# thu-ml/zhusuan

Measured on NVIDIA H100. Metric: leapfrog-steps*chains/sec, higher is better.
Workload: dtype f32

## Files before the change

zhusuan_b200/csrc/hmc_dense_res.cu:

```cuda
#include "hmc_dense_epilogue.cuh"

namespace {

struct ResEpi {
  const __half* __restrict__ hi_cur; const __half* __restrict__ lo_cur;
  __half* __restrict__ hi_nxt; __half* __restrict__ lo_nxt;
  const __half* __restrict__ hi_cur_s; const __half* __restrict__ lo_cur_s;
  __half* __restrict__ hi_nxt_s; __half* __restrict__ lo_nxt_s;
  const float* __restrict__ p_in; float* __restrict__ p_out;
  float* __restrict__ lp_part; float* __restrict__ k_part;
  int64_t chains; int D;
  float sq, inv_sq, acc_scale;
  float rescale;
};

template <int MODE, int NEXT, int DC, bool SPARE>
__device__ __forceinline__ void epilogue_planes(const ResEpi& a, uint32_t trow, int n, bool n_ok,
                                                int64_t c0, int64_t part_row, int lane, float s2,
                                                float eps_over_m_sq, float inv_m, float b_n,
                                                float mu_n, float& qmax) {
  constexpr int NCOL = BN;
  const uint32_t D = DC ? (uint32_t)DC : (uint32_t)a.D;
  const int64_t chains = a.chains;
  const bool warp_n_ok = __all_sync(0xffffffffu, n_ok);
  const bool fast_tile = warp_n_ok && (c0 + NCOL <= chains);
  const int64_t off_t = c0 * (int64_t)D + n;
  const float* __restrict__ pin0 = a.p_in + off_t;
  float* __restrict__ po0 = a.p_out + off_t;
  const unsigned short* __restrict__ hc0 =
      reinterpret_cast<const unsigned short*>(a.hi_cur) + off_t;
  const unsigned short* __restrict__ lc0 =
      reinterpret_cast<const unsigned short*>(a.lo_cur) + off_t;
  __half* __restrict__ hn0 = NEXT ? a.hi_nxt + off_t : nullptr;
  __half* __restrict__ ln0 = NEXT ? a.lo_nxt + off_t : nullptr;
  __half* __restrict__ hs0 = SPARE ? a.hi_nxt_s + off_t : nullptr;
  __half* __restrict__ ls0 = SPARE ? a.lo_nxt_s + off_t : nullptr;

  auto element = [&](float acc, float p, uint32_t hl, float& pn, float& lpv, float& kv,
                     float& Qn) {
    const float Q = __half2float(__ushort_as_half((unsigned short)(hl & 0xFFFFu))) +
                    __half2float(__ushort_as_half((unsigned short)(hl >> 16)));
    const float g = b_n - a.acc_scale * acc;
    pn = fmaf(s2, g, p);
    if (MODE >= 1) lpv = (Q * a.inv_sq - mu_n) * g;
    if (MODE >= 2) kv = pn * pn * inv_m;
    if (NEXT) Qn = fmaf(eps_over_m_sq, pn, Q);
  };

  if (fast_tile) {
    auto load = [&](float* pe, uint32_t* he, int c) {
      const size_t cb = (size_t)c * D;
#pragma unroll
      for (int j = 0; j < 16; ++j) {
        pe[j] = __ldcg(pin0 + cb + (uint32_t)j * D);
        const uint32_t h = __ldcg(hc0 + cb + (uint32_t)j * D);
        const uint32_t l = __ldcg(lc0 + cb + (uint32_t)j * D);
        he[j] = h | (l << 16);
      }
    };
    float ss_a = 0.f, ss_b = 0.f;
    auto compute = [&](const uint32_t* v, const float* pe, const uint32_t* he, int c, float& ss) {
      const size_t cb = (size_t)c * D;
      float lpv[MODE >= 1 ? 16 : 1], kv[MODE >= 2 ? 16 : 1];
#pragma unroll
      for (int j = 0; j < 16; j += 2) {
        float pn[2], lp1[2] = {0.f, 0.f}, k1[2] = {0.f, 0.f}, Qn[2] = {0.f, 0.f};
#pragma unroll
        for (int t = 0; t < 2; ++t) {
          element(__uint_as_float(v[j + t]), pe[j + t], he[j + t], pn[t], lp1[t], k1[t], Qn[t]);
          po0[cb + (uint32_t)(j + t) * D] = pn[t];
          if (MODE >= 1) lpv[j + t] = lp1[t];
          if (MODE >= 2) kv[j + t] = k1[t];
          if (NEXT && !SPARE) ss = fmaf(Qn[t], Qn[t], ss);
          if (SPARE) qmax = fmaxf(qmax, fabsf(Qn[t]));
        }
        if (NEXT) {
          const __half2 h2 = __floats2half2_rn(Qn[0], Qn[1]);
          const float2 hf = __half22float2(h2);
          const __half2 l2 = __floats2half2_rn(Qn[0] - hf.x, Qn[1] - hf.y);
          hn0[cb + (uint32_t)j * D] = __low2half(h2);
          hn0[cb + (uint32_t)(j + 1) * D] = __high2half(h2);
          ln0[cb + (uint32_t)j * D] = __low2half(l2);
          ln0[cb + (uint32_t)(j + 1) * D] = __high2half(l2);
        }
        if (SPARE) {
          const float x0 = Qn[0] * a.rescale, x1 = Qn[1] * a.rescale;
          const __half2 h2 = __floats2half2_rn(x0, x1);
          const float2 hf = __half22float2(h2);
          const __half2 l2 = __floats2half2_rn(x0 - hf.x, x1 - hf.y);
          hs0[cb + (uint32_t)j * D] = __low2half(h2);
          hs0[cb + (uint32_t)(j + 1) * D] = __high2half(h2);
          ls0[cb + (uint32_t)j * D] = __low2half(l2);
          ls0[cb + (uint32_t)(j + 1) * D] = __high2half(l2);
        }
      }
      if (MODE >= 1) {
        const float sum = warp_transpose_sum16(lpv, lane);
        if (lane < 16) a.lp_part[part_row + c0 + c + lane] = sum;
      }
      if (MODE >= 2) {
        const float sum = warp_transpose_sum16(kv, lane);
        if (lane < 16) a.k_part[part_row + c0 + c + lane] = sum;
      }
    };
    float pa[16], pb[16];
    uint32_t ha[16], hb[16], va[16], vb[16];
    load(pa, ha, 0);
#pragma unroll 1
    for (int c = 0; c < NCOL; c += 32) {
      load(pb, hb, c + 16);
      acc_ld16(trow + 4u * (uint32_t)c, va);
      compute(va, pa, ha, c, ss_a);
      if (c + 32 < NCOL) load(pa, ha, c + 32);
      acc_ld16(trow + 4u * (uint32_t)(c + 16), vb);
      compute(vb, pb, hb, c + 16, ss_b);
    }
    if (NEXT && !SPARE) {
      const float norm = sqrtf(ss_a + ss_b) * (1.f + 0x1p-10f);
      qmax = fmaxf(qmax, norm == norm ? norm : INFINITY);
    }
  } else {
#pragma unroll 1
    for (int c = 0; c < NCOL; c += 16) {
      uint32_t v[16];
      acc_ld16(trow + 4u * (uint32_t)c, v);
      const int64_t cbase = c0 + c;
      if (cbase < chains) {
        const size_t cb = (size_t)c * D;
        float lpv[MODE >= 1 ? 16 : 1], kv[MODE >= 2 ? 16 : 1];
#pragma unroll
        for (int j = 0; j < 16; ++j) {
          const bool ok = n_ok && cbase + j < chains;
          float p = 0.f;
          uint32_t hl = 0u;
          if (ok) {
            p = __ldcg(pin0 + cb + (uint32_t)j * D);
            hl = (uint32_t)__ldcg(hc0 + cb + (uint32_t)j * D) |
                 ((uint32_t)__ldcg(lc0 + cb + (uint32_t)j * D) << 16);
          }
          float pn, lp1 = 0.f, k1 = 0.f, Qn = 0.f;
          element(__uint_as_float(v[j]), p, hl, pn, lp1, k1, Qn);
          const __half hh = __float2half_rn(Qn);
          const __half ll = __float2half_rn(Qn - __half2float(hh));
          if (NEXT && ok) qmax = fmaxf(qmax, fabsf(Qn));
          if (MODE >= 1) lpv[j] = ok ? lp1 : 0.f;
          if (MODE >= 2) kv[j] = ok ? k1 : 0.f;
          if (ok) {
            po0[cb + (uint32_t)j * D] = pn;
            if (NEXT) {
              hn0[cb + (uint32_t)j * D] = hh;
              ln0[cb + (uint32_t)j * D] = ll;
            }
            if (SPARE) {
              const float x = Qn * a.rescale;
              const __half hs = __float2half_rn(x);
              hs0[cb + (uint32_t)j * D] = hs;
              ls0[cb + (uint32_t)j * D] = __float2half_rn(x - __half2float(hs));
            }
          }
        }
        if (MODE >= 1) {
          const float sum = warp_transpose_sum16(lpv, lane);
          if (lane < 16 && cbase + lane < chains) a.lp_part[part_row + cbase + lane] = sum;
        }
        if (MODE >= 2) {
          const float sum = warp_transpose_sum16(kv, lane);
          if (lane < 16 && cbase + lane < chains) a.k_part[part_row + cbase + lane] = sum;
        }
      }
    }
  }
}


__device__ __forceinline__ int& producer_spare_in() {
  __shared__ int spare_in;
  return spare_in;
}

template <int MODE, int NEXT, int DC, int CX, int CY>
struct ResW {
  static constexpr int KIND = 1, RB = 64, MNA = 0, MNB = 0;
  static constexpr int CLUSTER = CX * CY;
  static constexpr int KE = RB / 2;
  static constexpr uint32_t TX = Cfg<RB>::STAGE;
  CUtensorMap m_phi, m_plo, m_qhi, m_qlo, m_shi, m_slo;
  ResEpi ea;
  const float* bvec; const float* mu; const float* mass; const float* state;
  float* scales;
  float p_scale;
  int n_blk, D_rt, pass;
  struct EpiState { float qmax = 0.f; };

  __device__ __forceinline__ int D() const { return DC ? DC : D_rt; }
  __host__ __device__ __forceinline__ int64_t units() const {
    return ((ea.chains + BN - 1) / BN) * (int64_t)n_blk;
  }
  __device__ __forceinline__ void tile(int64_t u, int& nb, int64_t& cb) const {
    const uint64_t cu = (uint64_t)u / CLUSTER;
    const int r = (int)((uint64_t)u % CLUSTER);
    const uint32_t nbx = (uint32_t)(n_blk / CX);
    nb = (int)(cu % nbx) * CX + r % CX;
    cb = (int64_t)(cu / nbx) * CY + r / CX;
  }
  __device__ __forceinline__ void kb_range(int64_t, int& kb0, int& kb1) const {
    kb0 = 0;
    kb1 = D() / KE;
  }
  __device__ __forceinline__ void prefetch() const {
    tma_prefetch_desc(&m_phi); tma_prefetch_desc(&m_plo);
    tma_prefetch_desc(&m_qhi); tma_prefetch_desc(&m_qlo);
    tma_prefetch_desc(&m_shi); tma_prefetch_desc(&m_slo);
    producer_spare_in() = plane_spare_in(scales, pass);
  }
  __device__ __forceinline__ void load(int64_t u, int kb, uint32_t sa, uint32_t fb) const {
    using C = Cfg<RB>;
    int nb;
    int64_t cb;
    tile(u, nb, cb);
    const int n0 = nb * BM;
    const int c0 = (int)cb * BN;
    const bool s = producer_spare_in() != 0;
    const CUtensorMap* qh = s ? &m_shi : &m_qhi;
    const CUtensorMap* ql = s ? &m_slo : &m_qlo;
    const int r = (int)(u % CLUSTER), rx = r % CX, ry = r / CX;
    if constexpr (CY == 1) {
      tma_load_2d(sa, &m_phi, fb, kb * KE, n0);
      tma_load_2d(sa + C::A_TILE, &m_plo, fb, kb * KE, n0);
    } else {
      constexpr int rows = BM / CY;
      uint16_t mask = 0;
#pragma unroll
      for (int y = 0; y < CY; ++y) mask |= (uint16_t)(1u << (y * CX + rx));
      const uint32_t o = (uint32_t)(ry * rows * RB);
      tma_load_2d_mc(sa + o, &m_phi, fb, kb * KE, n0 + ry * rows, mask);
      tma_load_2d_mc(sa + C::A_TILE + o, &m_plo, fb, kb * KE, n0 + ry * rows, mask);
    }
    if constexpr (CX == 1) {
      tma_load_2d(sa + 2 * C::A_TILE, qh, fb, kb * KE, c0);
      tma_load_2d(sa + 2 * C::A_TILE + C::B_TILE, ql, fb, kb * KE, c0);
    } else {
      constexpr int rows = BN / CX;
      const uint16_t mask = (uint16_t)(((1u << CX) - 1u) << (ry * CX));
      const uint32_t o = (uint32_t)(rx * rows * RB);
      tma_load_2d_mc(sa + 2 * C::A_TILE + o, qh, fb, kb * KE, c0 + rx * rows, mask);
      tma_load_2d_mc(sa + 2 * C::A_TILE + C::B_TILE + o, ql, fb, kb * KE, c0 + rx * rows, mask);
    }
  }
  __device__ __forceinline__ float sq_alt(float eps, float sq) const {
    return next_plane_scale(scales, pass, eps, mul(eps, p_scale), sq);
  }
  __device__ __forceinline__ void epilogue(int64_t u, uint32_t trow, int quarter, int lane,
                                           EpiState& st) const {
    int nb;
    int64_t cb;
    tile(u, nb, cb);
    const int n = nb * BM + quarter * 32 + lane;
    const int64_t c0 = cb * BN;
    const bool n_ok = n < D();
    const float eps = state[ZSB_ST_EPS_USED];
    const float s2 = mul(eps, p_scale);
    const bool spare_in = plane_spare_in(scales, pass);
    const float sq = plane_scale_in(scales, pass);
    const float m_n = n_ok ? mass[n] : 1.f;
    const float eps_over_m_sq = mul(fdiv(eps, m_n), sq);
    const float inv_m = fdiv(1.f, m_n);
    const float b_n = (n_ok && bvec) ? bvec[n] : 0.f;
    const float mu_n = (n_ok && mu) ? mu[n] : 0.f;
    const int64_t part_row = (int64_t)(nb * 4 + quarter) * ea.chains;
    ResEpi a = ea;
    if (spare_in) {
      a.hi_cur = ea.hi_cur_s;
      a.lo_cur = ea.lo_cur_s;
    }
    a.sq = sq;
    a.inv_sq = fdiv(1.f, sq);
    a.acc_scale = 1.f / (scales[3] * sq);
    a.rescale = NEXT ? sq_alt(eps, sq) * a.inv_sq : 1.f;
    if (a.rescale == 1.f)
      epilogue_planes<MODE, NEXT, DC, false>(a, trow, n, n_ok, c0, part_row, lane, s2,
                                             eps_over_m_sq, inv_m, b_n, mu_n, st.qmax);
    else
      epilogue_planes<MODE, NEXT, DC, true>(a, trow, n, n_ok, c0, part_row, lane, s2,
                                            eps_over_m_sq, inv_m, b_n, mu_n, st.qmax);
  }
  __device__ __forceinline__ void epi_finish(EpiState& st, int quarter, int lane) const {
    if (!NEXT) return;
    const float sq = plane_scale_in(scales, pass);
    const float alt = sq_alt(state[ZSB_ST_EPS_USED], sq);
    publish_plane_scale(scales, pass, sq, alt, st.qmax * (1.f / sq),
                        alt != sq && !(st.qmax < kHalfOverflow), quarter, lane);
  }
};

constexpr int RES_CX = 2, RES_CY = 2;

template <int DC, int CX, int CY>
int res_pass(const CUtensorMap& phi, const CUtensorMap& plo, const CUtensorMap& qhi,
             const CUtensorMap& qlo, const CUtensorMap& shi, const CUtensorMap& slo,
             const ResEpi& ea, const float* bvec, const float* mu, const float* mass,
             const float* state, float* scales, int pass, float p_scale, int n_blk, int D,
             int mode, cudaStream_t st) {
  if (mode == 1) {
    const ResW<1, 1, DC, CX, CY> w{phi, plo, qhi, qlo, shi, slo, ea, bvec, mu, mass, state,
                                   scales, p_scale, n_blk, D, pass};
    return tc_launch(w, st, "hmc_dense_resident");
  }
  if (mode == 0) {
    const ResW<0, 1, DC, CX, CY> w{phi, plo, qhi, qlo, shi, slo, ea, bvec, mu, mass, state,
                                   scales, p_scale, n_blk, D, pass};
    return tc_launch(w, st, "hmc_dense_resident");
  }
  const ResW<2, 0, DC, CX, CY> w{phi, plo, qhi, qlo, shi, slo, ea, bvec, mu, mass, state, scales,
                                 p_scale, n_blk, D, pass};
  return tc_launch(w, st, "hmc_dense_resident");
}

template <int DC>
int res_pass(bool cluster, const CUtensorMap& phi, const CUtensorMap& plo, const CUtensorMap& qhi,
             const CUtensorMap& qlo, const CUtensorMap& shi, const CUtensorMap& slo,
             const ResEpi& ea, const float* bvec, const float* mu, const float* mass,
             const float* state, float* scales, int pass, float p_scale, int n_blk, int D,
             int mode, cudaStream_t st) {
  return cluster ? res_pass<DC, RES_CX, RES_CY>(phi, plo, qhi, qlo, shi, slo, ea, bvec, mu, mass,
                                                state, scales, pass, p_scale, n_blk, D, mode, st)
                 : res_pass<DC, 1, 1>(phi, plo, qhi, qlo, shi, slo, ea, bvec, mu, mass, state,
                                      scales, pass, p_scale, n_blk, D, mode, st);
}

__global__ void __launch_bounds__(256) select_planes_kernel(float* __restrict__ q,
                                                            const __half* __restrict__ planes,
                                                            const __half* __restrict__ spare,
                                                            const float* __restrict__ record,
                                                            const int32_t* __restrict__ accept,
                                                            int64_t chains, int64_t D) {
  const bool use_spare = __float_as_uint(record[3]) != 0u;
  const float inv_sq = 1.f / record[use_spare ? 1 : 0];
  if (use_spare) planes = spare;
  const int lane = threadIdx.x & 31;
  const int n8 = (int)(D >> 3);
  const int64_t wstride = (int64_t)gridDim.x * 8;
  for (int64_t c = (int64_t)blockIdx.x * 8 + (threadIdx.x >> 5); c < chains; c += wstride) {
    if (!accept[c]) continue;
    const uint4* __restrict__ hi = reinterpret_cast<const uint4*>(planes + c * D);
    const uint4* __restrict__ lo = reinterpret_cast<const uint4*>(planes + (chains + c) * D);
    float4* __restrict__ qr = reinterpret_cast<float4*>(q + c * D);
    for (int i0 = lane; i0 < n8; i0 += 128) {
      uint4 h[4], l[4];
#pragma unroll
      for (int u = 0; u < 4; ++u) {
        const int i = i0 + 32 * u;
        if (i < n8) { h[u] = __ldcs(hi + i); l[u] = __ldcs(lo + i); }
      }
#pragma unroll
      for (int u = 0; u < 4; ++u) {
        const int i = i0 + 32 * u;
        if (i < n8) {
          const uint32_t hw[4] = {h[u].x, h[u].y, h[u].z, h[u].w};
          const uint32_t lw[4] = {l[u].x, l[u].y, l[u].z, l[u].w};
          float o[8];
#pragma unroll
          for (int k = 0; k < 4; ++k) {
            const float2 hf = __half22float2(*reinterpret_cast<const __half2*>(&hw[k]));
            const float2 lf = __half22float2(*reinterpret_cast<const __half2*>(&lw[k]));
            o[2 * k] = (hf.x + lf.x) * inv_sq;
            o[2 * k + 1] = (hf.y + lf.y) * inv_sq;
          }
          qr[2 * i] = make_float4(o[0], o[1], o[2], o[3]);
          qr[2 * i + 1] = make_float4(o[4], o[5], o[6], o[7]);
        }
      }
    }
  }
}

}

int zsb_dense_res_h16_launch(void* planes0, void* planes1, void* spare0, void* spare1,
                             const float* p0, float* pw,
                             const void* P_h16, const void* P_l16, float* scales,
                             const float* bvec, const float* mu, const float* mass,
                             const float* state, float* lp0_part, float* lp1_part, float* k_part,
                             int64_t chains, int D, int L, cudaStream_t st) {
  if (D % 64 != 0 || D < 64 || L < 1 || chains <= 0 || chains >= (1LL << 31)) {
    zsb_set_error("dense_res: needs D %% 64 == 0, n_leapfrogs >= 1");
    return ZSB_ERR_INVALID;
  }
  if (planes0 == planes1 || !spare0 || !spare1 || spare0 == spare1) {
    zsb_set_error("dense_res: planes1, spare0 and spare1 must be separate work buffers");
    return ZSB_ERR_INVALID;
  }
  const int n_blk = (D + BM - 1) / BM;
  const int64_t c_blk = (chains + BN - 1) / BN;
  const bool cluster = n_blk % RES_CX == 0 && c_blk % RES_CY == 0;
  const uint32_t p_box = cluster ? BM / RES_CY : BM, q_box = cluster ? BN / RES_CX : BN;
  CUtensorMap phi, plo, qhi[2], qlo[2], shi[2], slo[2];
  int rc;
  constexpr int RB = ResW<0, 1, 0, 1, 1>::RB;
  if ((rc = make_map(&phi, P_h16, (uint64_t)D, (uint64_t)D, p_box, RB, 1))) return rc;
  if ((rc = make_map(&plo, P_l16, (uint64_t)D, (uint64_t)D, p_box, RB, 1))) return rc;
  __half* pl[2] = {reinterpret_cast<__half*>(planes0), reinterpret_cast<__half*>(planes1)};
  __half* sp[2] = {reinterpret_cast<__half*>(spare0), reinterpret_cast<__half*>(spare1)};
  const int64_t plane = chains * (int64_t)D;
  for (int b = 0; b < 2; ++b) {
    if ((rc = make_map(&qhi[b], pl[b], (uint64_t)chains, (uint64_t)D, q_box, RB, 1))) return rc;
    if ((rc = make_map(&qlo[b], pl[b] + plane, (uint64_t)chains, (uint64_t)D, q_box, RB, 1)))
      return rc;
    if ((rc = make_map(&shi[b], sp[b], (uint64_t)chains, (uint64_t)D, q_box, RB, 1))) return rc;
    if ((rc = make_map(&slo[b], sp[b] + plane, (uint64_t)chains, (uint64_t)D, q_box, RB, 1)))
      return rc;
  }
  for (int i = 0; i <= L; ++i) {
    const bool last = i == L;
    const int buf = i & 1;
    const ResEpi ea{pl[buf], pl[buf] + plane, pl[buf ^ 1], pl[buf ^ 1] + plane,
                    sp[buf], sp[buf] + plane, sp[buf ^ 1], sp[buf ^ 1] + plane,
                    i == 0 ? p0 : pw, pw, i == 0 ? lp0_part : lp1_part, k_part, chains, D,
                    1.f, 1.f, 1.f, 1.f};
    const int mode = last ? 2 : (i == 0 ? 1 : 0);
    const float p_scale = (i > 0 && !last) ? 1.f : 0.5f;
    rc = (D == 1024)
             ? res_pass<1024>(cluster, phi, plo, qhi[buf], qlo[buf], shi[buf], slo[buf], ea, bvec,
                              mu, mass, state, scales, i, p_scale, n_blk, D, mode, st)
             : res_pass<0>(cluster, phi, plo, qhi[buf], qlo[buf], shi[buf], slo[buf], ea, bvec, mu,
                           mass, state, scales, i, p_scale, n_blk, D, mode, st);
    if (rc != ZSB_OK) return rc;
  }
  return ZSB_OK;
}

int zsb_dense_select_planes_launch(float* q, const void* planes, const void* spare,
                                   const float* record, const int32_t* accept, int64_t chains,
                                   int64_t D, cudaStream_t st) {
  ZSB_REQUIRE(D % 8 == 0, "zsb_dense_select_planes: D must be a multiple of 8");
  int64_t blocks = zsb_ceil_div(chains, 8);
  if (blocks > ZSB_NUM_SMS * 16) blocks = ZSB_NUM_SMS * 16;
  if (blocks < 1) blocks = 1;
  select_planes_kernel<<<(unsigned)blocks, 256, 0, st>>>(
      q, reinterpret_cast<const __half*>(planes), reinterpret_cast<const __half*>(spare), record,
      accept, chains, D);
  return zsb_check_launch("hmc_select_planes");
}
```

zhusuan_b200/csrc/tc_common.cuh:

```cuda
#pragma once
#include "common.cuh"
#include <cuda.h>
#include <cuda_fp16.h>

namespace {

constexpr int BM = 128;
constexpr int BN = 128;
constexpr int NUM_EPI_WARPS = 4;
constexpr int PRODUCER_WARP = 4;
constexpr int EPI_WARP0 = 5;
constexpr int NUM_THREADS = 32 * (EPI_WARP0 + NUM_EPI_WARPS);
constexpr int ACC_LD = BN + 4;
constexpr int ACC_BYTES = BM * ACC_LD * 4;
constexpr int STAGE_BUDGET = 128 * 1024;
constexpr long long WAIT_TIMEOUT_CYCLES = 4000000000LL;

template <int RB>
struct Cfg {
  static constexpr int A_TILE = BM * RB;
  static constexpr int B_TILE = BN * RB;
  static constexpr int STAGE = 2 * A_TILE + 2 * B_TILE;
  static constexpr int STAGES = STAGE_BUDGET / STAGE;
  static constexpr int SMEM = STAGES * STAGE + ACC_BYTES + 128 + 1024;
};

__device__ __forceinline__ uint32_t smem_u32(const void* p) {
  return (uint32_t)__cvta_generic_to_shared(p);
}
__device__ __forceinline__ void mbar_init(uint32_t bar, uint32_t count) {
  asm volatile("mbarrier.init.shared::cta.b64 [%0], %1;" ::"r"(bar), "r"(count) : "memory");
}
__device__ __forceinline__ void mbar_expect_tx(uint32_t bar, uint32_t bytes) {
  asm volatile("mbarrier.arrive.expect_tx.shared::cta.b64 _, [%0], %1;" ::"r"(bar), "r"(bytes)
               : "memory");
}
__device__ __forceinline__ void mbar_arrive(uint32_t bar) {
  asm volatile("mbarrier.arrive.shared::cta.b64 _, [%0];" ::"r"(bar) : "memory");
}
__device__ __forceinline__ bool mbar_try_wait(uint32_t bar, uint32_t parity) {
  uint32_t ok;
  asm volatile(
      "{\n\t.reg .pred P1;\n\t"
      "mbarrier.try_wait.parity.shared::cta.b64 P1, [%1], %2;\n\t"
      "selp.b32 %0, 1, 0, P1;\n\t}"
      : "=r"(ok)
      : "r"(bar), "r"(parity)
      : "memory");
  return ok != 0;
}
__device__ __forceinline__ void mbar_wait(uint32_t bar, uint32_t parity) {
  if (mbar_try_wait(bar, parity)) return;
  const long long t0 = clock64();
  while (!mbar_try_wait(bar, parity))
    if (clock64() - t0 > WAIT_TIMEOUT_CYCLES) __trap();
}
__device__ __forceinline__ void mbar_spin(uint32_t bar, uint32_t parity) {
  while (!mbar_try_wait(bar, parity)) {
  }
}
__device__ __forceinline__ void tma_load_2d(uint32_t dst, const CUtensorMap* map, uint32_t bar,
                                            int c0, int c1) {
  asm volatile(
      "cp.async.bulk.tensor.2d.shared::cluster.global.mbarrier::complete_tx::bytes"
      " [%0], [%1, {%3, %4}], [%2];"
      ::"r"(dst), "l"(map), "r"(bar), "r"(c0), "r"(c1)
      : "memory");
}
__device__ __forceinline__ void tma_load_2d_mc(uint32_t dst, const CUtensorMap* map, uint32_t bar,
                                               int c0, int c1, uint16_t mask) {
  asm volatile(
      "cp.async.bulk.tensor.2d.shared::cluster.global.mbarrier::complete_tx::bytes"
      ".multicast::cluster [%0], [%1, {%3, %4}], [%2], %5;"
      ::"r"(dst), "l"(map), "r"(bar), "r"(c0), "r"(c1), "h"(mask)
      : "memory");
}
__device__ __forceinline__ void mbar_arrive_cluster(uint32_t bar, uint32_t cta) {
  asm volatile(
      "{\n\t.reg .b32 rb;\n\t"
      "mapa.shared::cluster.u32 rb, %0, %1;\n\t"
      "mbarrier.arrive.shared::cluster.b64 _, [rb];\n\t}"
      ::"r"(bar), "r"(cta)
      : "memory");
}
__device__ __forceinline__ void cluster_sync() {
  asm volatile("barrier.cluster.arrive.release;\n\tbarrier.cluster.wait.acquire;" ::: "memory");
}
__device__ __forceinline__ void tma_prefetch_desc(const CUtensorMap* map) {
  asm volatile("prefetch.tensormap [%0];" ::"l"(map) : "memory");
}

template <int MN, int RB>
__device__ __forceinline__ uint64_t gmma_desc(uint32_t saddr) {
  uint64_t d = (uint64_t)((saddr & 0x3FFFF) >> 4);
  if (MN) {
    d |= (uint64_t)(8192 >> 4) << 16;
    d |= (uint64_t)(1024 >> 4) << 32;
    d |= (uint64_t)1 << 62;
  } else {
    d |= (uint64_t)1 << 16;
    d |= (uint64_t)((8 * RB) >> 4) << 32;
    d |= (uint64_t)(RB == 128 ? 1 : 2) << 62;
  }
  return d;
}
__device__ __forceinline__ void wgmma_fence() {
  asm volatile("wgmma.fence.sync.aligned;" ::: "memory");
}
__device__ __forceinline__ void wgmma_commit() {
  asm volatile("wgmma.commit_group.sync.aligned;" ::: "memory");
}
template <int N>
__device__ __forceinline__ void wgmma_wait() {
  asm volatile("wgmma.wait_group.sync.aligned %0;" ::"n"(N) : "memory");
}
__device__ __forceinline__ void wgmma_tf32(float (&d)[64], uint64_t da, uint64_t db) {
  asm volatile(
      "{\n\t.reg .pred p;\n\tsetp.ne.b32 p, 1, 0;\n\t"
      "wgmma.mma_async.sync.aligned.m64n128k8.f32.tf32.tf32 {%0, %1, %2, %3, %4, %5, %6, %7, %8, %9, %10, %11, %12, %13, %14, %15, %16, %17, %18, %19, %20, %21, %22, %23, %24, %25, %26, %27, %28, %29, %30, %31, %32, %33, %34, %35, %36, %37, %38, %39, %40, %41, %42, %43, %44, %45, %46, %47, %48, %49, %50, %51, %52, %53, %54, %55, %56, %57, %58, %59, %60, %61, %62, %63}, %64, %65, p, 1, 1;\n\t}"
      : "+f"(d[0]), "+f"(d[1]), "+f"(d[2]), "+f"(d[3]), "+f"(d[4]), "+f"(d[5]), "+f"(d[6]), "+f"(d[7]), "+f"(d[8]), "+f"(d[9]), "+f"(d[10]), "+f"(d[11]), "+f"(d[12]), "+f"(d[13]), "+f"(d[14]), "+f"(d[15]), "+f"(d[16]), "+f"(d[17]), "+f"(d[18]), "+f"(d[19]), "+f"(d[20]), "+f"(d[21]), "+f"(d[22]), "+f"(d[23]), "+f"(d[24]), "+f"(d[25]), "+f"(d[26]), "+f"(d[27]), "+f"(d[28]), "+f"(d[29]), "+f"(d[30]), "+f"(d[31]), "+f"(d[32]), "+f"(d[33]), "+f"(d[34]), "+f"(d[35]), "+f"(d[36]), "+f"(d[37]), "+f"(d[38]), "+f"(d[39]), "+f"(d[40]), "+f"(d[41]), "+f"(d[42]), "+f"(d[43]), "+f"(d[44]), "+f"(d[45]), "+f"(d[46]), "+f"(d[47]), "+f"(d[48]), "+f"(d[49]), "+f"(d[50]), "+f"(d[51]), "+f"(d[52]), "+f"(d[53]), "+f"(d[54]), "+f"(d[55]), "+f"(d[56]), "+f"(d[57]), "+f"(d[58]), "+f"(d[59]), "+f"(d[60]), "+f"(d[61]), "+f"(d[62]), "+f"(d[63])
      : "l"(da), "l"(db));
}
template <int TA, int TB>
__device__ __forceinline__ void wgmma_f16(float (&d)[64], uint64_t da, uint64_t db) {
  asm volatile(
      "{\n\t.reg .pred p;\n\tsetp.ne.b32 p, 1, 0;\n\t"
      "wgmma.mma_async.sync.aligned.m64n128k16.f32.f16.f16 {%0, %1, %2, %3, %4, %5, %6, %7, %8, %9, %10, %11, %12, %13, %14, %15, %16, %17, %18, %19, %20, %21, %22, %23, %24, %25, %26, %27, %28, %29, %30, %31, %32, %33, %34, %35, %36, %37, %38, %39, %40, %41, %42, %43, %44, %45, %46, %47, %48, %49, %50, %51, %52, %53, %54, %55, %56, %57, %58, %59, %60, %61, %62, %63}, %64, %65, p, 1, 1, %66, %67;\n\t}"
      : "+f"(d[0]), "+f"(d[1]), "+f"(d[2]), "+f"(d[3]), "+f"(d[4]), "+f"(d[5]), "+f"(d[6]), "+f"(d[7]), "+f"(d[8]), "+f"(d[9]), "+f"(d[10]), "+f"(d[11]), "+f"(d[12]), "+f"(d[13]), "+f"(d[14]), "+f"(d[15]), "+f"(d[16]), "+f"(d[17]), "+f"(d[18]), "+f"(d[19]), "+f"(d[20]), "+f"(d[21]), "+f"(d[22]), "+f"(d[23]), "+f"(d[24]), "+f"(d[25]), "+f"(d[26]), "+f"(d[27]), "+f"(d[28]), "+f"(d[29]), "+f"(d[30]), "+f"(d[31]), "+f"(d[32]), "+f"(d[33]), "+f"(d[34]), "+f"(d[35]), "+f"(d[36]), "+f"(d[37]), "+f"(d[38]), "+f"(d[39]), "+f"(d[40]), "+f"(d[41]), "+f"(d[42]), "+f"(d[43]), "+f"(d[44]), "+f"(d[45]), "+f"(d[46]), "+f"(d[47]), "+f"(d[48]), "+f"(d[49]), "+f"(d[50]), "+f"(d[51]), "+f"(d[52]), "+f"(d[53]), "+f"(d[54]), "+f"(d[55]), "+f"(d[56]), "+f"(d[57]), "+f"(d[58]), "+f"(d[59]), "+f"(d[60]), "+f"(d[61]), "+f"(d[62]), "+f"(d[63])
      : "l"(da), "l"(db), "n"(TA), "n"(TB));
}

__device__ __forceinline__ void acc_ld16(uint32_t addr, uint32_t v[16]) {
#pragma unroll
  for (int i = 0; i < 4; ++i)
    asm volatile("ld.shared.v4.b32 {%0, %1, %2, %3}, [%4];"
                 : "=r"(v[4 * i]), "=r"(v[4 * i + 1]), "=r"(v[4 * i + 2]), "=r"(v[4 * i + 3])
                 : "r"(addr + 16u * i));
}

__device__ __forceinline__ float warp_transpose_sum16(float v[16], int lane) {
#pragma unroll
  for (int i = 0; i < 16; ++i) v[i] += __shfl_xor_sync(0xffffffffu, v[i], 16);
#pragma unroll
  for (int o = 8, cnt = 16; o >= 1; o >>= 1, cnt >>= 1) {
    const bool upper = (lane & o) != 0;
#pragma unroll
    for (int i = 0; i < cnt / 2; ++i) {
      const float keep = upper ? v[i + cnt / 2] : v[i];
      const float send = upper ? v[i] : v[i + cnt / 2];
      v[i] = keep + __shfl_xor_sync(0xffffffffu, send, o);
    }
  }
  return v[0];
}

template <int KIND, int RB, int MNA, int MNB, int ZLO = 0>
__device__ __forceinline__ void mma_kblock(float (&d)[2][64], uint32_t sa) {
  using C = Cfg<RB>;
#pragma unroll
  for (int k = 0; k < RB / 32; ++k) {
    const uint32_t bo = MNB ? (uint32_t)k * 2048u : (uint32_t)k * 32u;
    const uint64_t b_hi = gmma_desc<MNB, RB>(sa + 2 * C::A_TILE + bo);
    const uint64_t b_lo = gmma_desc<MNB, RB>(sa + 2 * C::A_TILE + C::B_TILE + bo);
#pragma unroll
    for (int mh = 0; mh < 2; ++mh) {
      const uint32_t ao = MNA ? (uint32_t)mh * 8192u + (uint32_t)k * 2048u
                              : (uint32_t)(mh * 64 * RB) + (uint32_t)k * 32u;
      const uint64_t a_hi = gmma_desc<MNA, RB>(sa + ao);
      const uint64_t a_lo = gmma_desc<MNA, RB>(sa + C::A_TILE + ao);
      if (KIND == 0) {
        wgmma_tf32(d[mh], a_lo, b_hi);
        wgmma_tf32(d[mh], a_hi, b_lo);
        wgmma_tf32(d[mh], a_hi, b_hi);
      } else {
        if (!(ZLO & 1)) wgmma_f16<MNA, MNB>(d[mh], a_lo, b_hi);
        if (!(ZLO & 2)) wgmma_f16<MNA, MNB>(d[mh], a_hi, b_lo);
        wgmma_f16<MNA, MNB>(d[mh], a_hi, b_hi);
      }
    }
  }
}

template <class W, class = void>
struct ClusterOf {
  static constexpr int value = 1;
};
template <class W>
struct ClusterOf<W, decltype((void)W::CLUSTER)> {
  static constexpr int value = W::CLUSTER;
};

template <class W, class = void>
struct ZloOf {
  static constexpr int value = 0;
};
template <class W>
struct ZloOf<W, decltype((void)W::ZLO)> {
  static constexpr int value = W::ZLO;
};

template <class W>
__global__ void __launch_bounds__(NUM_THREADS, 1) tc_pipeline_kernel(const __grid_constant__ W w) {
  using C = Cfg<W::RB>;
  constexpr int CS = ClusterOf<W>::value;
  extern __shared__ uint8_t smem_raw[];
  const uint32_t smem_base = (smem_u32(smem_raw) + 1023u) & ~1023u;
  const uint32_t acc_base = smem_base + C::STAGES * C::STAGE;
  const uint32_t bars = acc_base + ACC_BYTES;
  const uint32_t full_bar = bars;
  const uint32_t empty_bar = bars + 8 * C::STAGES;
  const uint32_t tfull_bar = bars + 16 * C::STAGES;
  const uint32_t tempty_bar = tfull_bar + 8;

  const int warp = __shfl_sync(0xffffffffu, (int)(threadIdx.x >> 5), 0);
  const int lane = threadIdx.x & 31;
  const int64_t n_units = w.units();

  if (threadIdx.x == 0) {
    for (int s = 0; s < C::STAGES; ++s) {
      mbar_init(full_bar + 8 * s, 1);
      mbar_init(empty_bar + 8 * s, CS);
    }
    mbar_init(tfull_bar, 128);
    mbar_init(tempty_bar, 32 * NUM_EPI_WARPS);
    asm volatile("fence.mbarrier_init.release.cluster;" ::: "memory");
  }
  if constexpr (CS > 1)
    cluster_sync();
  else
    __syncthreads();
  auto release = [&](int s) {
    if constexpr (CS > 1) {
#pragma unroll
      for (int r = 0; r < CS; ++r) mbar_arrive_cluster(empty_bar + 8 * s, (uint32_t)r);
    } else {
      mbar_arrive(empty_bar + 8 * s);
    }
  };

  if (warp < 4) {
    const int tid = threadIdx.x;
    float d[2][64];
    int stage = 0;
    uint32_t phase = 0, acc_phase = 0;
    for (int64_t u = blockIdx.x; u < n_units; u += gridDim.x) {
      int kb0, kb1;
      w.kb_range(u, kb0, kb1);
#pragma unroll
      for (int mh = 0; mh < 2; ++mh)
#pragma unroll
        for (int i = 0; i < 64; ++i) d[mh][i] = 0.f;
      int prev = -1;
      for (int kb = kb0; kb < kb1; ++kb) {
        const uint32_t sa = smem_base + stage * C::STAGE;
        mbar_spin(full_bar + 8 * stage, phase);
        wgmma_fence();
        mma_kblock<W::KIND, W::RB, W::MNA, W::MNB, ZloOf<W>::value>(d, sa);
        wgmma_commit();
        wgmma_wait<1>();
        if (prev >= 0 && tid == 0) release(prev);
        prev = stage;
        if (++stage == C::STAGES) { stage = 0; phase ^= 1; }
      }
      wgmma_wait<0>();
      if (prev >= 0 && tid == 0) release(prev);
      mbar_wait(tempty_bar, acc_phase ^ 1);
      const int row = 16 * (tid >> 5) + ((tid & 31) >> 2);
      const int col = 2 * (tid & 3);
#pragma unroll
      for (int mh = 0; mh < 2; ++mh)
#pragma unroll
        for (int j = 0; j < 16; ++j) {
          const uint32_t a0 = acc_base + (uint32_t)(((64 * mh + row) * ACC_LD + 8 * j + col) * 4);
          asm volatile("st.shared.v2.f32 [%0], {%1, %2};" ::"r"(a0), "f"(d[mh][4 * j]),
                       "f"(d[mh][4 * j + 1]) : "memory");
          asm volatile("st.shared.v2.f32 [%0], {%1, %2};" ::"r"(a0 + 8u * ACC_LD * 4u),
                       "f"(d[mh][4 * j + 2]), "f"(d[mh][4 * j + 3]) : "memory");
        }
      mbar_arrive(tfull_bar);
      acc_phase ^= 1;
    }
  } else if (warp == PRODUCER_WARP) {
    if (lane == 0) {
      w.prefetch();
      int stage = 0;
      uint32_t phase = 0;
      for (int64_t u = blockIdx.x; u < n_units; u += gridDim.x) {
        int kb0, kb1;
        w.kb_range(u, kb0, kb1);
        for (int kb = kb0; kb < kb1; ++kb) {
          mbar_wait(empty_bar + 8 * stage, phase ^ 1);
          const uint32_t fb = full_bar + 8 * stage;
          mbar_expect_tx(fb, W::TX);
          w.load(u, kb, smem_base + stage * C::STAGE, fb);
          if (++stage == C::STAGES) { stage = 0; phase ^= 1; }
        }
      }
    }
  } else {
    const int quarter = warp - EPI_WARP0;
    const uint32_t trow = acc_base + (uint32_t)((quarter * 32 + lane) * ACC_LD * 4);
    typename W::EpiState st;
    uint32_t acc_phase = 0;
    for (int64_t u = blockIdx.x; u < n_units; u += gridDim.x) {
      mbar_wait(tfull_bar, acc_phase);
      w.epilogue(u, trow, quarter, lane, st);
      __syncwarp();
      mbar_arrive(tempty_bar);
      acc_phase ^= 1;
    }
    w.epi_finish(st, quarter, lane);
  }
  if constexpr (CS > 1) cluster_sync();
}

template <class W>
int tc_launch(const W& w, cudaStream_t st, const char* what) {
  constexpr int CS = ClusterOf<W>::value;
  static const cudaError_t attr = cudaFuncSetAttribute(
      tc_pipeline_kernel<W>, cudaFuncAttributeMaxDynamicSharedMemorySize, Cfg<W::RB>::SMEM);
  if (attr != cudaSuccess) {
    zsb_set_error("%s: cudaFuncSetAttribute: %s", what, cudaGetErrorString(attr));
    return ZSB_ERR_CUDA;
  }
  if constexpr (CS > 1) {
    const int64_t units = w.units();
    if (units < 1 || units % CS != 0) {
      zsb_set_error("%s: %lld units do not tile by clusters of %d", what, (long long)units, CS);
      return ZSB_ERR_INVALID;
    }
    cudaLaunchAttribute cl[1];
    cl[0].id = cudaLaunchAttributeClusterDimension;
    cl[0].val.clusterDim.x = CS;
    cl[0].val.clusterDim.y = 1;
    cl[0].val.clusterDim.z = 1;
    cudaLaunchConfig_t cfg = {};
    cfg.blockDim = dim3(NUM_THREADS);
    cfg.dynamicSmemBytes = Cfg<W::RB>::SMEM;
    cfg.stream = st;
    cfg.attrs = cl;
    cfg.numAttrs = 1;
    static int max_clusters = 0;
    if (max_clusters < 1) {
      cfg.gridDim = dim3(CS);
      const cudaError_t e =
          cudaOccupancyMaxActiveClusters(&max_clusters, tc_pipeline_kernel<W>, &cfg);
      if (e != cudaSuccess || max_clusters < 1) {
        zsb_set_error("%s: no cluster of %d CTAs fits (%s)", what, CS, cudaGetErrorString(e));
        max_clusters = 0;
        return ZSB_ERR_CUDA;
      }
    }
    int64_t grid = (int64_t)max_clusters * CS;
    if (grid > units) grid = units;
    cfg.gridDim = dim3((unsigned)grid);
    const cudaError_t e = cudaLaunchKernelEx(&cfg, tc_pipeline_kernel<W>, w);
    if (e != cudaSuccess) {
      zsb_set_error("%s: cudaLaunchKernelEx: %s", what, cudaGetErrorString(e));
      return ZSB_ERR_CUDA;
    }
    return zsb_check_launch(what);
  } else {
    int dev = 0, sms = ZSB_NUM_SMS;
    cudaGetDevice(&dev);
    cudaDeviceGetAttribute(&sms, cudaDevAttrMultiProcessorCount, dev);
    int64_t grid = w.units();
    if (grid > sms) grid = sms;
    if (grid < 1) grid = 1;
    tc_pipeline_kernel<W><<<(unsigned)grid, NUM_THREADS, Cfg<W::RB>::SMEM, st>>>(w);
    return zsb_check_launch(what);
  }
}

typedef CUresult (*EncodeTiledFn)(CUtensorMap*, CUtensorMapDataType, cuuint32_t, void*,
                                  const cuuint64_t*, const cuuint64_t*, const cuuint32_t*,
                                  const cuuint32_t*, CUtensorMapInterleave, CUtensorMapSwizzle,
                                  CUtensorMapL2promotion, CUtensorMapFloatOOBfill);

EncodeTiledFn get_encode_fn() {
  static EncodeTiledFn fn = nullptr;
  if (!fn) {
    void* p = nullptr;
    cudaDriverEntryPointQueryResult qres;
    if (cudaGetDriverEntryPoint("cuTensorMapEncodeTiled", &p, cudaEnableDefault, &qres) !=
            cudaSuccess || qres != cudaDriverEntryPointSuccess)
      return nullptr;
    fn = (EncodeTiledFn)p;
  }
  return fn;
}

int make_map(CUtensorMap* map, const void* base, uint64_t rows, uint64_t cols, uint32_t box_rows,
             int rb, int half_elems = 0) {
  EncodeTiledFn enc = get_encode_fn();
  if (!enc) {
    zsb_set_error("tc: cuTensorMapEncodeTiled unavailable");
    return ZSB_ERR_CUDA;
  }
  const int esz = half_elems ? 2 : 4;
  cuuint64_t dims[2] = {cols, rows};
  cuuint64_t strides[1] = {cols * esz};
  cuuint32_t box[2] = {(cuuint32_t)(rb / esz), box_rows};
  cuuint32_t estr[2] = {1, 1};
  CUresult r = enc(map, half_elems ? CU_TENSOR_MAP_DATA_TYPE_FLOAT16 : CU_TENSOR_MAP_DATA_TYPE_FLOAT32,
                   2, (void*)base, dims, strides, box, estr,
                   CU_TENSOR_MAP_INTERLEAVE_NONE,
                   rb == 128 ? CU_TENSOR_MAP_SWIZZLE_128B : CU_TENSOR_MAP_SWIZZLE_64B,
                   CU_TENSOR_MAP_L2_PROMOTION_L2_256B, CU_TENSOR_MAP_FLOAT_OOB_FILL_NONE);
  if (r != CUDA_SUCCESS) {
    zsb_set_error("tc: cuTensorMapEncodeTiled failed (%d)", (int)r);
    return ZSB_ERR_CUDA;
  }
  return ZSB_OK;
}

}
```

Baseline: 70.80 million.

## Retune resident cluster shape and operand ring depth, add pass profiling hooks

Switches the resident dense pass cluster from 2x2 to 2x1. The operand-ring stage count is now fixed per K-block size (2 stages for RB=128, 5 otherwise) instead of being derived from a 128KB budget, with smaller alignment padding for the non-128 case. It also adds compile-time-gated clock64 profiling counters and a readback helper, and swaps the mbarrier timeout from SM cycles to globaltimer nanoseconds. Cluster multicast sharing and pipeline depth change, which alters load reuse and shared memory use per CTA.

After: 73.60 million, median of 6. +4.0%, better.

```diff
diff --git a/zhusuan_b200/csrc/hmc_dense_res.cu b/zhusuan_b200/csrc/hmc_dense_res.cu
--- a/zhusuan_b200/csrc/hmc_dense_res.cu
+++ b/zhusuan_b200/csrc/hmc_dense_res.cu
@@ -293,7 +293,7 @@
   }
 };
 
-constexpr int RES_CX = 2, RES_CY = 2;
+constexpr int RES_CX = 2, RES_CY = 1;
 
 template <int DC, int CX, int CY>
 int res_pass(const CUtensorMap& phi, const CUtensorMap& plo, const CUtensorMap& qhi,
@@ -429,6 +429,17 @@
   return ZSB_OK;
 }
 
+#ifdef ZSB_PASS_PROFILE
+extern "C" int zsb_pass_profile_read(unsigned long long* host, int ctas) {
+  if (ctas < 0 || ctas > PASS_PROF_CTAS) return ZSB_ERR_INVALID;
+  const size_t bytes = sizeof(unsigned long long) * PASS_PROF_SLOTS * (size_t)ctas;
+  if (cudaMemcpyFromSymbol(host, g_pass_prof, bytes) != cudaSuccess) return ZSB_ERR_CUDA;
+  static unsigned long long zeros[PASS_PROF_CTAS * PASS_PROF_SLOTS];
+  if (cudaMemcpyToSymbol(g_pass_prof, zeros, sizeof(zeros)) != cudaSuccess) return ZSB_ERR_CUDA;
+  return ZSB_OK;
+}
+#endif
+
 int zsb_dense_select_planes_launch(float* q, const void* planes, const void* spare,
                                    const float* record, const int32_t* accept, int64_t chains,
                                    int64_t D, cudaStream_t st) {
diff --git a/zhusuan_b200/csrc/tc_common.cuh b/zhusuan_b200/csrc/tc_common.cuh
--- a/zhusuan_b200/csrc/tc_common.cuh
+++ b/zhusuan_b200/csrc/tc_common.cuh
@@ -13,16 +13,46 @@
 constexpr int NUM_THREADS = 32 * (EPI_WARP0 + NUM_EPI_WARPS);
 constexpr int ACC_LD = BN + 4;
 constexpr int ACC_BYTES = BM * ACC_LD * 4;
-constexpr int STAGE_BUDGET = 128 * 1024;
-constexpr long long WAIT_TIMEOUT_CYCLES = 4000000000LL;
+constexpr unsigned long long WAIT_TIMEOUT_NS = 2000000000ULL;
+
+enum PassProfSlot {
+  PROF_MMA_TOTAL,
+  PROF_MMA_FULL,
+  PROF_MMA_TEMPTY,
+  PROF_MMA_STORE,
+  PROF_PROD_EMPTY,
+  PROF_EPI_TFULL,
+  PROF_EPI_UNIT,
+  PROF_UNITS,
+  PASS_PROF_SLOTS
+};
+constexpr int PASS_PROF_CTAS = 1024;
+#ifdef ZSB_PASS_PROFILE
+constexpr bool kPassProfile = true;
+__device__ unsigned long long g_pass_prof[PASS_PROF_CTAS * PASS_PROF_SLOTS];
+#else
+constexpr bool kPassProfile = false;
+#endif
+__device__ __forceinline__ long long prof_clock() {
+  if constexpr (kPassProfile) return clock64();
+  return 0;
+}
+__device__ __forceinline__ void prof_add(int slot, long long v) {
+#ifdef ZSB_PASS_PROFILE
+  if (blockIdx.x < PASS_PROF_CTAS)
+    atomicAdd(&g_pass_prof[blockIdx.x * PASS_PROF_SLOTS + slot], (unsigned long long)v);
+#endif
+}
 
 template <int RB>
 struct Cfg {
   static constexpr int A_TILE = BM * RB;
   static constexpr int B_TILE = BN * RB;
   static constexpr int STAGE = 2 * A_TILE + 2 * B_TILE;
-  static constexpr int STAGES = STAGE_BUDGET / STAGE;
-  static constexpr int SMEM = STAGES * STAGE + ACC_BYTES + 128 + 1024;
+  static constexpr int STAGES = RB == 128 ? 2 : 5;
+  static constexpr int ALIGN = RB == 128 ? 1024 : 512;
+  static constexpr int SMEM = STAGES * STAGE + ACC_BYTES + 128 + ALIGN;
+  static_assert(SMEM <= 227 * 1024, "operand ring exceeds shared memory");
 };
 
 __device__ __forceinline__ uint32_t smem_u32(const void* p) {
@@ -49,11 +79,16 @@
       : "memory");
   return ok != 0;
 }
+__device__ __forceinline__ unsigned long long global_ns() {
+  unsigned long long t;
+  asm volatile("mov.u64 %0, %%globaltimer;" : "=l"(t));
+  return t;
+}
 __device__ __forceinline__ void mbar_wait(uint32_t bar, uint32_t parity) {
   if (mbar_try_wait(bar, parity)) return;
-  const long long t0 = clock64();
+  const unsigned long long t0 = global_ns();
   while (!mbar_try_wait(bar, parity))
-    if (clock64() - t0 > WAIT_TIMEOUT_CYCLES) __trap();
+    if (global_ns() - t0 > WAIT_TIMEOUT_NS) __trap();
 }
 __device__ __forceinline__ void mbar_spin(uint32_t bar, uint32_t parity) {
   while (!mbar_try_wait(bar, parity)) {
@@ -204,7 +239,7 @@
   using C = Cfg<W::RB>;
   constexpr int CS = ClusterOf<W>::value;
   extern __shared__ uint8_t smem_raw[];
-  const uint32_t smem_base = (smem_u32(smem_raw) + 1023u) & ~1023u;
+  const uint32_t smem_base = (smem_u32(smem_raw) + (C::ALIGN - 1)) & ~(uint32_t)(C::ALIGN - 1);
   const uint32_t acc_base = smem_base + C::STAGES * C::STAGE;
   const uint32_t bars = acc_base + ACC_BYTES;
   const uint32_t full_bar = bars;
@@ -243,6 +278,8 @@
     float d[2][64];
     int stage = 0;
     uint32_t phase = 0, acc_phase = 0;
+    const long long t_begin = prof_clock();
+    long long t_full = 0, t_tempty = 0, t_store = 0, units = 0;
     for (int64_t u = blockIdx.x; u < n_units; u += gridDim.x) {
       int kb0, kb1;
       w.kb_range(u, kb0, kb1);
@@ -253,7 +290,9 @@
       int prev = -1;
       for (int kb = kb0; kb < kb1; ++kb) {
         const uint32_t sa = smem_base + stage * C::STAGE;
+        const long long t0 = prof_clock();
         mbar_spin(full_bar + 8 * stage, phase);
+        t_full += prof_clock() - t0;
         wgmma_fence();
         mma_kblock<W::KIND, W::RB, W::MNA, W::MNB, ZloOf<W>::value>(d, sa);
         wgmma_commit();
@@ -264,7 +303,10 @@
       }
       wgmma_wait<0>();
       if (prev >= 0 && tid == 0) release(prev);
+      const long long t1 = prof_clock();
       mbar_wait(tempty_bar, acc_phase ^ 1);
+      const long long t2 = prof_clock();
+      t_tempty += t2 - t1;
       const int row = 16 * (tid >> 5) + ((tid & 31) >> 2);
       const int col = 2 * (tid & 3);
 #pragma unroll
@@ -279,35 +321,57 @@
         }
       mbar_arrive(tfull_bar);
       acc_phase ^= 1;
+      t_store += prof_clock() - t2;
+      ++units;
+    }
+    if (kPassProfile && tid == 0) {
+      prof_add(PROF_MMA_TOTAL, prof_clock() - t_begin);
+      prof_add(PROF_MMA_FULL, t_full);
+      prof_add(PROF_MMA_TEMPTY, t_tempty);
+      prof_add(PROF_MMA_STORE, t_store);
+      prof_add(PROF_UNITS, units);
     }
   } else if (warp == PRODUCER_WARP) {
     if (lane == 0) {
       w.prefetch();
       int stage = 0;
       uint32_t phase = 0;
+      long long t_empty = 0;
       for (int64_t u = blockIdx.x; u < n_units; u += gridDim.x) {
         int kb0, kb1;
         w.kb_range(u, kb0, kb1);
         for (int kb = kb0; kb < kb1; ++kb) {
+          const long long t0 = prof_clock();
           mbar_wait(empty_bar + 8 * stage, phase ^ 1);
+          t_empty += prof_clock() - t0;
           const uint32_t fb = full_bar + 8 * stage;
           mbar_expect_tx(fb, W::TX);
           w.load(u, kb, smem_base + stage * C::STAGE, fb);
           if (++stage == C::STAGES) { stage = 0; phase ^= 1; }
         }
       }
+      if (kPassProfile) prof_add(PROF_PROD_EMPTY, t_empty);
     }
   } else {
     const int quarter = warp - EPI_WARP0;
     const uint32_t trow = acc_base + (uint32_t)((quarter * 32 + lane) * ACC_LD * 4);
     typename W::EpiState st;
     uint32_t acc_phase = 0;
+    long long t_tfull = 0, t_unit = 0;
     for (int64_t u = blockIdx.x; u < n_units; u += gridDim.x) {
+      const long long t0 = prof_clock();
       mbar_wait(tfull_bar, acc_phase);
+      const long long t1 = prof_clock();
       w.epilogue(u, trow, quarter, lane, st);
       __syncwarp();
       mbar_arrive(tempty_bar);
       acc_phase ^= 1;
+      t_tfull += t1 - t0;
+      t_unit += prof_clock() - t1;
+    }
+    if (kPassProfile && quarter == 0 && lane == 0) {
+      prof_add(PROF_EPI_TFULL, t_tfull);
+      prof_add(PROF_EPI_UNIT, t_unit);
     }
     w.epi_finish(st, quarter, lane);
   }
```
